# RobotVisionHKA/LiFCal

Measured on AMD Instinct MI355X. Metric: micro-image obs/sec through Jacobian+Schur at 1M obs, higher is better.
Workload: dtype f64; 1 GPU; metric_web: 334 frames, 24720 points, 999994 micro-image observations, window 10, config 0xf06 (2 radial + tangential, mlCenterAdj, Cauchy(0.5), refine poses+points); lens_selection=reference generator (lifcal_mla_project), obs_per_gpu=999994, n_reduced=2021, deterministic=False

## Files before the change

lifcal_amd/csrc/sweep3.hpp:

```cpp
#pragma once

namespace lifcal {

template <int NR, bool TAN, bool ADJ, int WR, class ET = double>
__global__ __launch_bounds__(128 * WR, 2) void k_sweep3(Dev d, double radius, int mode) {
  constexpr bool F32 = sizeof(ET) == 4;
  constexpr int NC = 5 + NR + (TAN ? 2 : 0);
  constexpr int NCC = NC * (NC + 1) / 2;
  constexpr int HV = 6 + 2 * NC + 2;
  constexpr uint32_t LP = 64u * WR;
  constexpr uint32_t NT = 2u * LP;
  static_assert(HV * LP <= V2Lds::zd_for(LP), "hand-off buffer must fit the Z matrix");
  if (radius < 0.0 && d.lm[LM_TERMINATION] != 0.0) return;
  extern __shared__ __attribute__((aligned(16))) double sm[];
  const V2Lds lay(d.v2_nfmax, true, LP);
  const uint32_t NFm = lay.nfm, vlen = 6 * NFm + NCMAX + 3;
  double* Spp = sm; double* Scp = sm + lay.off_cp; double* Scc = sm + lay.off_cc;
  double* vgB = sm + lay.off_vec; double* vhd = vgB + vlen; double* vrhs = vhd + vlen;
  double* Fr = sm + lay.off_fr;
  double* slab = sm + lay.off_slab;
  double* Zd = sm + lay.off_zd;
  double* misc = sm + lay.off_misc;
  uint32_t* pidl = (uint32_t*)(misc + MISC_DOUBLES);
  unsigned short* colinfo = (unsigned short*)(misc + MISC_DOUBLES + 32);
  uint32_t flip = 0;
#ifndef LIFCAL_NO_ROLE_FLIP
  if (WR == 2) flip = (__builtin_amdgcn_s_getreg(6 | (0 << 6) | (7 << 11)) != 0) ? LP : 0u;
#endif
  const uint32_t tid = threadIdx.x ^ flip, lane = tid & 63u, w = tid >> 6;
  const bool role_b = w >= (uint32_t)WR;
  const uint32_t wl = w & (uint32_t)(WR - 1);
  const uint32_t t256 = tid & (LP - 1u);
  const uint32_t b = blockIdx.x;
  const uint32_t flo = d.blk_flo[b], nf = d.blk_nf[b];
  const uint32_t ncol = 6 * nf + NC + 1, ncolp = (ncol + 15u) & ~15u;
  const uint32_t zs = ncolp + 2;
  const CamConsts c = *d.camc;
#ifdef LIFCAL_STAMPS
  unsigned long long st_acc[16] = {0, 0, 0, 0, 0, 0, 0, 0, 0, 0, 0, 0, 0, 0, 0, 0}, st_last = 0;
  if (tid == 0 || tid == LP) { asm volatile("s_memtime %0\n\ts_waitcnt lgkmcnt(0)" : "=s"(st_last) :: "memory"); }
#define STAMPB(i) do { if (tid == LP) { unsigned long long t_; asm volatile("s_memtime %0\n\ts_waitcnt lgkmcnt(0)" : "=s"(t_) :: "memory"); st_acc[i] += t_ - st_last; st_last = t_; } } while (0)
#else
#define STAMPB(i) do { } while (0)
#endif
  const uint32_t ps_begin = d.blk_pass0[b], ps_end = d.blk_pass0[b + 1];
  uint32_t nx_np = 0, nx_si = 0, nx_pt = 0, nx_fp = 0, nx_gid = 0, nx_r[2] = {0, 0};
  uint32_t vz;
  asm volatile("v_mov_b32 %0, 0" : "=v"(vz));
  auto fetch_pass = [&](uint32_t q) {
    nx_np = d.pass_np[q + vz];
    nx_si = d.v2_slot[(size_t)q * LP + t256]; nx_pt = d.v2f_pt[(size_t)q * LP + t256]; nx_gid = d.v2_gidx[(size_t)q * LP + t256];
    nx_r[0] = d.v2_tile_row0[q * WR + wl + vz]; nx_r[1] = d.v2_tile_row0[q * WR + wl + 1 + vz];
    nx_fp = d.v2_passpt[(size_t)q * 64 + (tid & 63u)];
  };
  if (ps_begin < ps_end) fetch_pass(ps_begin);
  { double2* z2 = reinterpret_cast<double2*>(sm); for (uint32_t i = tid; i < lay.off_slab / 2; i += NT) z2[i] = double2{0.0, 0.0}; }
  if (tid == 0 && (lay.off_slab & 1u)) sm[lay.off_slab - 1] = 0.0;
  if (tid < MISC_DOUBLES) misc[tid] = 0.0;
  for (uint32_t cI = tid; cI < ncolp; cI += NT)
    colinfo[cI] = (cI < 6 * nf) ? (unsigned short)(((cI / 6) << 8) | (cI % 6)) : (cI < ncol - 1 ? (unsigned short)(0x8000u | (cI - 6 * nf)) : (unsigned short)0xC000u);

  auto zero_slab = [&]() { for (uint32_t i = tid; i < lay.np_max * SLAB_STRIDE; i += NT) slab[i] = 0.0; };
  auto zero_zd = [&](uint32_t krows) { double2* z2 = reinterpret_cast<double2*>(Zd); for (uint32_t i = tid; i < (krows * zs) / 2; i += NT) z2[i] = double2{0.0, 0.0}; };
  auto z_phase = [&](uint32_t np) {
    const uint32_t nwc = ncol - 1;
    const uint32_t nth = NT / nwc > 0 ? NT / nwc : 1;
    const uint32_t gi = tid / nwc, cidx = tid - gi * nwc;
    if (gi < nth || nwc > NT) {
      for (uint32_t cc0 = cidx; cc0 < nwc; cc0 += (nwc > NT ? NT : nwc * nth)) {
#pragma unroll 4
        for (uint32_t lp = (nwc > NT ? 0 : gi); lp < np; lp += (nwc > NT ? 1 : nth)) {
          const double* acc = slab + lp * SLAB_STRIDE;
          double* z = Zd + (size_t)(3 * lp) * zs + cc0;
          const double w0 = z[0], w1 = z[zs], w2 = z[2 * zs];
          if (cc0 >= 6 * nf) {
            double* ga = d.ptacc + (size_t)pidl[lp] * 36 + 9 + (cc0 - 6 * nf);
            store_stream(ga, w0); store_stream(ga + NCMAX, w1); store_stream(ga + 2 * NCMAX, w2);
          }
          z[0] = acc[0] * w0; z[zs] = acc[1] * w0 + acc[3] * w1; z[2 * zs] = acc[2] * w0 + acc[4] * w1 + acc[5] * w2;
        }
      }
    }
  };
  struct LaneGeom { double R[9], Y[3], Gr[3][3]; };
  auto lane_geom = [&](uint32_t fr, uint32_t pt, LaneGeom& q) {
    const double* ft = d.ft + (size_t)fr * FRAME_STRIDE;
    const double* P = d.pts + 3 * (size_t)pt;
#pragma unroll
    for (int k = 0; k < 9; ++k) q.R[k] = ft[k];
    const double P0 = P[0], P1 = P[1], P2 = P[2];
#pragma unroll
    for (int k = 0; k < 3; ++k) q.Y[k] = q.R[3 * k] * P0 + q.R[3 * k + 1] * P1 + q.R[3 * k + 2] * P2;
    const double c0 = ft[12], s0 = ft[13], n0 = q.R[2], n1 = q.R[5], n2 = q.R[8];
    q.Gr[0][0] = 0.0;     q.Gr[0][1] = c0 * q.Y[2] - s0 * q.Y[1]; q.Gr[0][2] = n1 * q.Y[2] - n2 * q.Y[1];
    q.Gr[1][0] = -q.Y[2]; q.Gr[1][1] = s0 * q.Y[0];               q.Gr[1][2] = n2 * q.Y[0] - n0 * q.Y[2];
    q.Gr[2][0] = q.Y[1];  q.Gr[2][1] = -c0 * q.Y[0];              q.Gr[2][2] = n0 * q.Y[1] - n1 * q.Y[0];
  };
  const uint32_t frs = NFm * lay.nrep;
  struct RunMask { double m1, m2, m4, m8; bool head; };
  auto run_masks = [&](uint32_t cnt, uint32_t lf) {
    const int key = cnt > 0 ? (int)lf : (int)(0x7F000000u + lane);
    RunMask r;
    r.m1 = __builtin_amdgcn_update_dpp(-1, key, 0x101, 0xf, 0xf, false) == key ? 1.0 : 0.0;
    r.m2 = __builtin_amdgcn_update_dpp(-1, key, 0x102, 0xf, 0xf, false) == key ? 1.0 : 0.0;
    r.m4 = __builtin_amdgcn_update_dpp(-1, key, 0x104, 0xf, 0xf, false) == key ? 1.0 : 0.0;
    r.m8 = __builtin_amdgcn_update_dpp(-1, key, 0x108, 0xf, 0xf, false) == key ? 1.0 : 0.0;
    r.head = cnt > 0 && __builtin_amdgcn_update_dpp(-1, key, 0x111, 0xf, 0xf, false) != key;
    return r;
  };
  auto run_sum = [](double v, const RunMask& r) {
    auto shl = [](double x, auto ctrl) {
      const int lo = __double2loint(x), hi = __double2hiint(x);
      return __hiloint2double(__builtin_amdgcn_update_dpp(0, hi, decltype(ctrl)::value, 0xf, 0xf, true),
                              __builtin_amdgcn_update_dpp(0, lo, decltype(ctrl)::value, 0xf, 0xf, true));
    };
    v = fma(shl(v, std::integral_constant<int, 0x101>{}), r.m1, v);
    v = fma(shl(v, std::integral_constant<int, 0x102>{}), r.m2, v);
    v = fma(shl(v, std::integral_constant<int, 0x104>{}), r.m4, v);
    v = fma(shl(v, std::integral_constant<int, 0x108>{}), r.m8, v);
    return v;
  };
  uint32_t* hw_written = (uint32_t*)(misc + 4) + wl;
  uint32_t* hw_read = (uint32_t*)(misc + 4) + 4 + wl;
  uint32_t* eval_done = (uint32_t*)(misc + 3);
  const bool det = d.deterministic != 0;
  uint32_t* turn = (uint32_t*)(misc + 8) + (role_b ? 1 : 0);
  uint32_t my_turn = wl;
  auto wait_for = [](uint32_t* flag, uint32_t need) {
    while (__hip_atomic_load(flag, __ATOMIC_ACQUIRE, __HIP_MEMORY_SCOPE_WORKGROUP) < need) __builtin_amdgcn_s_sleep(2);
  };
  auto publish = [](uint32_t* flag, uint32_t value) {
    asm volatile("s_waitcnt lgkmcnt(0)" ::: "memory");
    __hip_atomic_store(flag, value, __ATOMIC_RELEASE, __HIP_MEMORY_SCOPE_WORKGROUP);
  };

  const uint32_t nmt = (ncol + 3u) >> 2, ntri = nmt * (nmt + 1) / 2;
  auto tri_decode = [](uint32_t t, uint32_t& mi, uint32_t& mj) {
    mi = (uint32_t)((sqrtf(8.0f * (float)t + 1.0f) - 1.0f) * 0.5f);
    while (mi * (mi + 1) / 2 > t) --mi;
    while ((mi + 1) * (mi + 2) / 2 <= t) ++mi;
    mj = t - mi * (mi + 1) / 2;
  };
  auto gemm_tile = [&](uint32_t mi, uint32_t mj, uint32_t kfirst, uint32_t kstep, uint32_t krows, double (&acc16)[4][4]) {
    const double* za = Zd + 4 * mi;
    const double* zb = Zd + 4 * mj;
    double2 cur[4][4];
#pragma unroll
    for (int r = 0; r < 4; ++r) {
      cur[r][0] = *reinterpret_cast<const double2*>(za + (size_t)(kfirst + r) * zs);
      cur[r][1] = *reinterpret_cast<const double2*>(za + (size_t)(kfirst + r) * zs + 2);
      cur[r][2] = *reinterpret_cast<const double2*>(zb + (size_t)(kfirst + r) * zs);
      cur[r][3] = *reinterpret_cast<const double2*>(zb + (size_t)(kfirst + r) * zs + 2);
    }
#pragma unroll 2
    for (uint32_t k0 = kfirst; k0 < krows; k0 += kstep) {
      double2 nxt[4][4];
      const uint32_t kn = (k0 + kstep < krows) ? k0 + kstep : k0;
#pragma unroll
      for (int r = 0; r < 4; ++r) {
        nxt[r][0] = *reinterpret_cast<const double2*>(za + (size_t)(kn + r) * zs);
        nxt[r][1] = *reinterpret_cast<const double2*>(za + (size_t)(kn + r) * zs + 2);
        nxt[r][2] = *reinterpret_cast<const double2*>(zb + (size_t)(kn + r) * zs);
        nxt[r][3] = *reinterpret_cast<const double2*>(zb + (size_t)(kn + r) * zs + 2);
      }
#pragma unroll
      for (int r = 0; r < 4; ++r) {
        const double av[4] = {cur[r][0].x, cur[r][0].y, cur[r][1].x, cur[r][1].y};
        const double bq[4] = {cur[r][2].x, cur[r][2].y, cur[r][3].x, cur[r][3].y};
#pragma unroll
        for (int i = 0; i < 4; ++i)
#pragma unroll
          for (int j = 0; j < 4; ++j) acc16[i][j] += av[i] * bq[j];
      }
#pragma unroll
      for (int r = 0; r < 4; ++r)
#pragma unroll
        for (int q = 0; q < 4; ++q) cur[r][q] = nxt[r][q];
    }
  };
  auto emit_tile = [&](uint32_t mi, uint32_t mj, const double (&acc16)[4][4]) {
#pragma unroll
    for (int i = 0; i < 4; ++i) {
      const uint32_t ci = 4 * mi + i;
      const uint32_t ii = colinfo[ci < ncolp ? ci : 0];
#pragma unroll
      for (int j = 0; j < 4; ++j) {
        const uint32_t cj = 4 * mj + j;
        const double dv = acc16[i][j];
        if (ci >= ncol || cj >= ncol || ci < cj) continue;
        const uint32_t jj = colinfo[cj];
        if (!(ii & 0x8000u)) {
          const uint32_t lfi = ii >> 8, lfj = jj >> 8;
          Spp[(size_t)(lfi * (lfi + 1) / 2 + lfj) * 36 + (ii & 0xFFu) * 6 + (jj & 0xFFu)] -= dv;
        } else if (!(ii & 0x4000u)) {
          const uint32_t jc = ii & 0xFFu;
          if (!(jj & 0x8000u)) Scp[(size_t)jc * 6 * NFm + cj] -= dv;
          else Scc[jc * (jc + 1) / 2 + (jj & 0xFFu)] -= dv;
        } else if (cj < ncol - 1) {
          if (!(jj & 0x8000u)) vrhs[cj] += dv; else vrhs[6 * NFm + (jj & 0xFFu)] += dv;
        }
      }
    }
  };
  const bool keep_tiles = (WR == 4) && (mode == 0) && ntri <= LP;
  const bool ksplit = keep_tiles && lay.has_bt();
  const bool share_tiles = (WR != 4) && (mode == 0);
  double* bt = sm + lay.off_bt;
  if (!role_b) {
    double cost = 0.0, lmant = 1.0; int lexp = 0;
    uint32_t hbase = 0;
    uint32_t passes_done = 0;
    uint32_t mi0 = 0, mj0 = 0;
    if (keep_tiles && tid < ntri) tri_decode(tid, mi0, mj0);
    double tacc[4][4];
#pragma unroll
    for (int i = 0; i < 4; ++i)
#pragma unroll
      for (int j = 0; j < 4; ++j) tacc[i][j] = 0.0;

    STAMP(14);
    for (uint32_t ps = ps_begin; ps < ps_end; ++ps) {
      const uint32_t np = __builtin_amdgcn_readfirstlane(nx_np);
      const uint32_t si = nx_si, pt = nx_pt, fp = nx_fp, gidx = nx_gid;
      const uint32_t row0 = __builtin_amdgcn_readfirstlane(nx_r[0]), kmax = __builtin_amdgcn_readfirstlane(nx_r[1]) - row0;
      if (ps + 1 < ps_end) fetch_pass(ps + 1);
      const uint32_t krows = (3 * np + 7u) & ~7u;
      const uint32_t cnt = si & 0xFFu, lf = (si >> 8) & 0xFFu, lp = (si >> 16) & 0xFFu;
      const uint32_t fr = flo + lf;
      const ET* obs_u = F32 ? reinterpret_cast<const ET*>(d.v2_du) : reinterpret_cast<const ET*>(d.v2_u);
      const ET* obs_v = F32 ? reinterpret_cast<const ET*>(d.v2_dv) : reinterpret_cast<const ET*>(d.v2_v);
      const ET* lens_tab = F32 ? reinterpret_cast<const ET*>(d.ltf) : reinterpret_cast<const ET*>(d.lt);
      double ftv[12], P0, P1, P2;
      {
        const double* ft = d.ft + (size_t)fr * FRAME_STRIDE;
        const double* P = d.pts + 3 * (size_t)pt;
#pragma unroll
        for (int i = 0; i < 12; ++i) ftv[i] = ft[i];
        P0 = P[0]; P1 = P[1]; P2 = P[2];
      }
      ET ua = 0, va = 0, ub = 0, vb = 0; uint32_t lb = 0, la = 0, l0 = 0;
      {
        const size_t at = (size_t)row0 * 64 + lane;
        const size_t at2 = ((size_t)row0 + (kmax > 1 ? 1u : 0u)) * 64 + lane;
        ua = obs_u[at]; va = obs_v[at]; l0 = d.v2_lens[at];
        ub = obs_u[at2]; vb = obs_v[at2]; lb = d.v2_lens[at2];
      }
      STAMP(12);
      zero_slab();
      STAMP(13);
      lds_barrier();
      STAMP(0);
      typename std::conditional<F32, GroupConsts2F, GroupConsts2>::type gcn;
      {
        const double Xc = ftv[0] * P0 + ftv[1] * P1 + ftv[2] * P2 + ftv[9], Yc = ftv[3] * P0 + ftv[4] * P1 + ftv[5] * P2 + ftv[10], Zc = ftv[6] * P0 + ftv[7] * P1 + ftv[8] * P2 + ftv[11];
        if constexpr (F32) group_prepare2f<ADJ>(c, Xc, Yc, Zc, gcn); else group_prepare2<ADJ>(c, Xc, Yc, Zc, gcn);
      }
      double A[6] = {0, 0, 0, 0, 0, 0}, bv[3] = {0, 0, 0};
      ET* hand = reinterpret_cast<ET*>(Zd) + t256;
      constexpr uint32_t HS = LP;
      ET Ln[LENS_STRIDE];
      double wn0 = 0.0, wn1 = 0.0;
      {
        const ET* L = lens_tab + (size_t)l0 * LENS_STRIDE;
#pragma unroll
        for (int i = 0; i < LENS_STRIDE; ++i) Ln[i] = L[i];
        if constexpr (F32) { wn0 = d.ltw[2 * (size_t)l0]; wn1 = d.ltw[2 * (size_t)l0 + 1]; }
      }
      typename std::conditional<F32, CamF, int>::type cf{};
      if constexpr (F32) cf = cam_to_float(c);
      auto step = [&](uint32_t k, ET& uc, ET& vc, uint32_t& lc, const uint32_t ln) {
        wait_for(hw_read, hbase + k);
        if (k < cnt) {
          const ET u = uc, v = vc;
          ET L[LENS_STRIDE];
#pragma unroll
          for (int i = 0; i < LENS_STRIDE; ++i) L[i] = Ln[i];
          ET r[2], Jq[2][3], Jc[2][NC];
          ET arg;
          if constexpr (F32) obs_eval2f_pk<NR, TAN, ADJ>(cf, gcn, L, wn0, wn1, u, v, d.robust != 0, r, Jq, Jc, arg);
          else obs_eval2<NR, TAN, ADJ>(c, gcn, L, u, v, d.robust != 0, r, Jq, Jc, arg);
#pragma unroll
          for (int a = 0; a < 2; ++a) {
#pragma unroll
            for (int j = 0; j < NC; ++j) hand[(6 + a * NC + j) * HS] = Jc[a][j];
#pragma unroll
            for (int i = 0; i < 3; ++i) hand[(a * 3 + i) * HS] = Jq[a][i];
            hand[(6 + 2 * NC + a) * HS] = r[a];
          }
          if (d.robust) { int ex; lmant = frexp(lmant * (double)arg, &ex); lexp += ex; }
          else cost += 0.5 * (double)arg;
#pragma unroll
          for (int a = 0; a < 2; ++a) {
            const double q0 = Jq[a][0], q1 = Jq[a][1], q2 = Jq[a][2], ra = r[a];
            A[0] += q0 * q0; A[1] += q0 * q1; A[2] += q0 * q2;
            A[3] += q1 * q1; A[4] += q1 * q2; A[5] += q2 * q2;
            bv[0] += q0 * ra; bv[1] += q1 * ra; bv[2] += q2 * ra;
          }
        }
        {
          const ET* Lp = lens_tab + (size_t)ln * LENS_STRIDE;
#pragma unroll
          for (int i = 0; i < LENS_STRIDE; ++i) Ln[i] = Lp[i];
          if constexpr (F32) { wn0 = d.ltw[2 * (size_t)ln]; wn1 = d.ltw[2 * (size_t)ln + 1]; }
          const uint32_t kk = (k + 2 < kmax) ? k + 2 : kmax - 1;
          const size_t at = ((size_t)row0 + kk) * 64 + lane;
          uc = obs_u[at]; vc = obs_v[at]; lc = d.v2_lens[at];
        }
        publish(hw_written, hbase + k + 1);
      };
      for (uint32_t k = 0; k < kmax; k += 2) {
        step(k, ua, va, la, lb);
        if (k + 1 < kmax) step(k + 1, ub, vb, lb, la);
      }
      hbase += kmax;
      LaneGeom q;
      { uint32_t fr2 = fr, pt2 = pt; asm volatile("" : "+v"(fr2), "+v"(pt2)); lane_geom(fr2, pt2, q); }
      asm volatile("" :: "v"(nx_si), "v"(nx_pt), "v"(nx_fp), "v"(nx_np), "v"(nx_gid), "v"(nx_r[0]), "v"(nx_r[1]));
      const double fsg0 = d.sigP[3 * (size_t)fp], fsg1 = d.sigP[3 * (size_t)fp + 1], fsg2 = d.sigP[3 * (size_t)fp + 2];
      STAMP(7);
      lds_barrier();
      if (mode == 0) zero_zd(krows);
      lds_barrier();
      asm volatile("" :: "v"(fsg0), "v"(fsg1), "v"(fsg2));
      if (det) wait_for(turn, my_turn);
      if (cnt > 0) {
        const double Am[3][3] = {{A[0], A[1], A[2]}, {A[1], A[3], A[4]}, {A[2], A[4], A[5]}};
        const double (&R)[9] = q.R; const double (&Gr)[3][3] = q.Gr;
        double AG[3][3], GAG[3][3];
#pragma unroll
        for (int i = 0; i < 3; ++i)
#pragma unroll
          for (int j = 0; j < 3; ++j) AG[i][j] = Am[i][0] * Gr[0][j] + Am[i][1] * Gr[1][j] + Am[i][2] * Gr[2][j];
#pragma unroll
        for (int i = 0; i < 3; ++i)
#pragma unroll
          for (int j = 0; j < 3; ++j) GAG[i][j] = Gr[0][i] * AG[0][j] + Gr[1][i] * AG[1][j] + Gr[2][i] * AG[2][j];
        RunMask rm = run_masks(cnt, lf);
        const bool fpose = d.frame_live[fr] != 0;
        rm.head = rm.head && fpose;
        double* fr_acc = Fr + lf;
        {
          int vi = 0;
#pragma unroll
          for (int a = 0; a < 6; ++a)
#pragma unroll
            for (int bb = 0; bb <= a; ++bb) {
              double v;
              if (a < 3) v = GAG[a][bb]; else if (bb < 3) v = AG[a - 3][bb]; else v = Am[a - 3][bb - 3];
              v = run_sum(v, rm);
              if (rm.head) atomicAdd(fr_acc + (size_t)vi * frs, v);
              ++vi;
            }
#pragma unroll
          for (int a = 0; a < 3; ++a) { const double v = run_sum(Gr[0][a] * bv[0] + Gr[1][a] * bv[1] + Gr[2][a] * bv[2], rm); if (rm.head) atomicAdd(fr_acc + (size_t)(21 + a) * frs, v); }
#pragma unroll
          for (int a = 0; a < 3; ++a) { const double v = run_sum(bv[a], rm); if (rm.head) atomicAdd(fr_acc + (size_t)(24 + a) * frs, v); }
        }
        double AR[3][3];
#pragma unroll
        for (int i = 0; i < 3; ++i)
#pragma unroll
          for (int j = 0; j < 3; ++j) AR[i][j] = Am[i][0] * R[j] + Am[i][1] * R[3 + j] + Am[i][2] * R[6 + j];
        double* acc = slab + lp * SLAB_STRIDE;
#pragma unroll
        for (int i = 0; i < 3; ++i) {
#pragma unroll
          for (int j = 0; j <= i; ++j) {
            const double u_ij = R[i] * AR[0][j] + R[3 + i] * AR[1][j] + R[6 + i] * AR[2][j];
            const int pos = (i == 0) ? 0 : (i == 1 ? (j == 0 ? 1 : 3) : (j == 0 ? 2 : (j == 1 ? 4 : 5)));
            atomicAdd(acc + pos, u_ij);
          }
        }
        if (mode == 0) {
          { double* ga = d.Av + (size_t)gidx * 6;
            store_stream(ga, A[0], A[1]); store_stream(ga + 2, A[2], A[3]); store_stream(ga + 4, A[4], A[5]); }
#pragma unroll
          for (int i = 0; i < 3; ++i) {
            atomicAdd(acc + 6 + i, R[i] * bv[0] + R[3 + i] * bv[1] + R[6 + i] * bv[2]);
            double* zrow = Zd + (size_t)(3 * lp + i) * zs + 6 * lf;
            double w6[6];
#pragma unroll
            for (int j = 0; j < 3; ++j) { w6[j] = R[i] * AG[0][j] + R[3 + i] * AG[1][j] + R[6 + i] * AG[2][j]; w6[3 + j] = R[i] * Am[0][j] + R[3 + i] * Am[1][j] + R[6 + i] * Am[2][j]; }
            const bool rot = (lp & 1u) != 0;
#pragma unroll
            for (int jj = 0; jj < 6; ++jj) {
              const double wv = rot ? w6[(jj + 1) % 6] : w6[jj];
              const uint32_t col = rot ? (uint32_t)((jj + 1) % 6) : (uint32_t)jj;
              if (fpose) atomicAdd(zrow + col, wv);
            }
          }
        }
      }
      if (det) { publish(turn, my_turn + 1); my_turn += (uint32_t)WR; }
      STAMP(6);
      asm volatile("s_waitcnt lgkmcnt(0)" ::: "memory");
      if (lane == 0) __hip_atomic_fetch_add(eval_done, 1u, __ATOMIC_RELAXED, __HIP_MEMORY_SCOPE_WORKGROUP);
      ++passes_done;
      if (w == 0) wait_for(eval_done, (uint32_t)WR * passes_done);
      STAMP(1);
      if (tid < np) {
        const uint32_t p = fp;
        pidl[tid] = p;
        double* acc = slab + tid * SLAB_STRIDE;
        double U0 = acc[0], U1 = acc[1], U2 = acc[2], U3 = acc[3], U4 = acc[4], U5 = acc[5];
        if (mode == 1) {
          double* ga = d.ptacc + (size_t)p * 36;
          store_stream(ga, U0); store_stream(ga + 3, U3); store_stream(ga + 5, U5);
        } else {
          const double g0 = acc[6], g1 = acc[7], g2 = acc[8];
          double lam[3];
          {
            const double h[3] = {U0, U3, U5}, sgv[3] = {fsg0, fsg1, fsg2};
#pragma unroll
            for (int k = 0; k < 3; ++k) { const double sg = sgv[k]; lam[k] = fmin(fmax(h[k] * sg * sg, d.lm_min), d.lm_max) / (lm_radius(d, radius) * sg * sg); }
          }
          U0 += lam[0]; U3 += lam[1]; U5 += lam[2];
          bool ok = U0 > 0.0;
          double i00 = rsqrt(U0);
          const double l10 = U1 * i00, l20 = U2 * i00;
          const double d11 = U3 - l10 * l10; ok = ok && (d11 > 0.0);
          double i11 = rsqrt(d11);
          const double l21 = (U4 - l20 * l10) * i11;
          const double d22 = U5 - l20 * l20 - l21 * l21; ok = ok && (d22 > 0.0);
          double i22 = rsqrt(d22);
          double m10 = -l10 * i00 * i11, m21 = -l21 * i11 * i22, m20 = -(l20 * i00 + l21 * m10) * i22;
          if (!ok) { i00 = i11 = i22 = m10 = m21 = m20 = 0.0; atomicAdd(misc + 1, 1.0); }
          double* gu = d.Uinv + 9 * (size_t)p;
          const double v00 = i00 * i00 + m10 * m10 + m20 * m20, v01 = m10 * i11 + m20 * m21, v02 = m20 * i22;
          const double v11 = i11 * i11 + m21 * m21, v12 = m21 * i22, v22 = i22 * i22;
          {
            const double vu[9] = {v00, v01, v02, v01, v11, v12, v02, v12, v22};
#pragma unroll
            for (int k = 0; k < 9; ++k) store_stream(gu + k, vu[k]);
          }
          double* gl = d.lamP + 3 * (size_t)p;
          double* ga = d.ptacc + (size_t)p * 36 + 6;
#pragma unroll
          for (int k = 0; k < 3; ++k) store_stream(gl + k, lam[k]);
          store_stream(ga, g0); store_stream(ga + 1, g1); store_stream(ga + 2, g2);
          const double gm = fmax(fabs(g0), fmax(fabs(g1), fabs(g2)));
          atomicMax((unsigned long long*)(misc + 2), (unsigned long long)__double_as_longlong(gm));
          acc[0] = i00; acc[1] = m10; acc[2] = m20; acc[3] = i11; acc[4] = m21; acc[5] = i22;
          double* z0 = Zd + (size_t)(3 * tid) * zs + (ncol - 1);
          z0[0] = i00 * g0; z0[zs] = m10 * g0 + i11 * g1; z0[2 * zs] = m20 * g0 + m21 * g1 + i22 * g2;
        }
      }
      lds_barrier();
      STAMP(2);
      if (mode == 0) {
        z_phase(np);
        lds_barrier();
        STAMP(3);
        if (keep_tiles) {
          if (tid < ntri) gemm_tile(mi0, mj0, 0, ksplit ? 8u : 4u, krows, tacc);
        } else {
          for (uint32_t t = tid; t < ntri; t += (share_tiles ? NT : LP)) {
            uint32_t mi, mj; tri_decode(t, mi, mj);
            double acc16[4][4];
#pragma unroll
            for (int i = 0; i < 4; ++i)
#pragma unroll
              for (int j = 0; j < 4; ++j) acc16[i][j] = 0.0;
            gemm_tile(mi, mj, 0, 4, krows, acc16);
            emit_tile(mi, mj, acc16);
          }
        }
      }
      lds_barrier();
      STAMP(4);
    }
    STAMP(8);
    if (keep_tiles && tid < ntri) {
      if (ksplit) {
#pragma unroll
        for (int i = 0; i < 4; ++i)
#pragma unroll
          for (int j = 0; j < 4; ++j) tacc[i][j] += bt[(i * 4 + j) * LP + tid];
      }
      uint32_t ci4[4], cj4[4];
#pragma unroll
      for (int i = 0; i < 4; ++i) { const uint32_t ci = 4 * mi0 + i, cj = 4 * mj0 + i; ci4[i] = colinfo[ci < ncolp ? ci : 0]; cj4[i] = colinfo[cj < ncolp ? cj : 0]; }
      uint32_t off[4][4]; double sg[4][4];
      const uint32_t dummy = lay.off_zd + 1024u + tid;
#pragma unroll
      for (int i = 0; i < 4; ++i)
#pragma unroll
        for (int j = 0; j < 4; ++j) {
          const uint32_t ci = 4 * mi0 + i, cj = 4 * mj0 + j, ii = ci4[i], jj = cj4[j];
          uint32_t o = dummy; double sgn = -1.0;
          if (!(ci >= ncol || cj >= ncol || ci < cj)) {
            if (!(ii & 0x8000u)) {
              const uint32_t lfi = ii >> 8, lfj = jj >> 8;
              o = (lfi * (lfi + 1) / 2 + lfj) * 36 + (ii & 0xFFu) * 6 + (jj & 0xFFu);
            } else if (!(ii & 0x4000u)) {
              const uint32_t jc = ii & 0xFFu;
              o = !(jj & 0x8000u) ? lay.off_cp + jc * 6 * NFm + cj : lay.off_cc + jc * (jc + 1) / 2 + (jj & 0xFFu);
            } else if (cj < ncol - 1) {
              o = lay.off_vec + 2 * vlen + (!(jj & 0x8000u) ? cj : 6 * NFm + (jj & 0xFFu));
              sgn = 1.0;
            }
          }
          off[i][j] = o; sg[i][j] = sgn;
        }
      double oldv[4][4];
#pragma unroll
      for (int i = 0; i < 4; ++i)
#pragma unroll
        for (int j = 0; j < 4; ++j) oldv[i][j] = sm[off[i][j]];
#pragma unroll
      for (int i = 0; i < 4; ++i)
#pragma unroll
        for (int j = 0; j < 4; ++j) sm[off[i][j]] = oldv[i][j] + sg[i][j] * tacc[i][j];
    }
    STAMP(9);
    if (d.robust) cost += 0.5 * c.loss_b * (log(lmant) + (double)lexp * 0.6931471805599453);
    cost = wave_sum_dpp(cost);
    if (det) wait_for(turn, my_turn);
    if (lane == 63) atomicAdd(misc + 0, cost);
    if (det) publish(turn, my_turn + 1);
    lds_barrier(); lds_barrier();
  } else {
    double cc[NCC], gc[NC];
    uint32_t hbase = 0;
#pragma unroll
    for (int i = 0; i < NCC; ++i) cc[i] = 0.0;
#pragma unroll
    for (int i = 0; i < NC; ++i) gc[i] = 0.0;
    for (uint32_t ps = ps_begin; ps < ps_end; ++ps) {
      const uint32_t np = __builtin_amdgcn_readfirstlane(nx_np);
      const uint32_t si = nx_si, pt = nx_pt;
      const uint32_t kmax = __builtin_amdgcn_readfirstlane(nx_r[1]) - __builtin_amdgcn_readfirstlane(nx_r[0]);
      if (ps + 1 < ps_end) fetch_pass(ps + 1);
      const uint32_t krows = (3 * np + 7u) & ~7u;
      zero_slab();
      lds_barrier();
      STAMPB(0);
      const uint32_t cnt = si & 0xFFu, lf = (si >> 8) & 0xFFu, lp = (si >> 16) & 0xFFu;
      double C[3][NC];
#pragma unroll
      for (int i = 0; i < 3; ++i)
#pragma unroll
        for (int j = 0; j < NC; ++j) C[i][j] = 0.0;
      const ET* hand = reinterpret_cast<const ET*>(Zd) + t256;
      constexpr uint32_t HS = LP;
      for (uint32_t k = 0; k < kmax; ++k) {
        wait_for(hw_written, hbase + k + 1);
        const bool live = k < cnt;
#pragma unroll
        for (int a = 0; a < 2; ++a) {
          double r = 0.0, Jq[3] = {0.0, 0.0, 0.0}, Jc[NC];
#pragma unroll
          for (int j = 0; j < NC; ++j) Jc[j] = 0.0;
          if (live) {
#pragma unroll
            for (int i = 0; i < 3; ++i) Jq[i] = hand[(a * 3 + i) * HS];
#pragma unroll
            for (int j = 0; j < NC; ++j) Jc[j] = hand[(6 + a * NC + j) * HS];
            r = hand[(6 + 2 * NC + a) * HS];
          }
          if (a == 1) publish(hw_read, hbase + k + 1);
          if (live) {
#pragma unroll
            for (int i = 0; i < 3; ++i)
#pragma unroll
              for (int j = 0; j < NC; ++j) C[i][j] += Jq[i] * Jc[j];
            int t = 0;
#pragma unroll
            for (int i = 0; i < NC; ++i) {
              gc[i] += Jc[i] * r;
#pragma unroll
              for (int j = 0; j <= i; ++j) cc[t++] += Jc[i] * Jc[j];
            }
          }
        }
      }
      hbase += kmax;
      asm volatile("" :: "v"(nx_si), "v"(nx_pt), "v"(nx_np), "v"(nx_r[0]), "v"(nx_r[1]));
      LaneGeom q;
      STAMPB(1);
      lane_geom(flo + lf, pt, q);
      lds_barrier();
      if (mode == 0) zero_zd(krows);
      lds_barrier();
      STAMPB(2);
      if (det) wait_for(turn, my_turn);
      if (mode == 0 && cnt > 0) {
        const double (&R)[9] = q.R; const double (&Gr)[3][3] = q.Gr;
#pragma unroll
        for (int i = 0; i < 3; ++i)
#pragma unroll
          for (int j = 0; j < NC; ++j) C[i][j] *= c.chm[j];
        RunMask rm = run_masks(cnt, lf);
        rm.head = rm.head && d.frame_live[flo + lf] != 0;
        double* fr_acc = Fr + lf;
#pragma unroll
        for (int j = 0; j < NC; ++j) {
#pragma unroll
          for (int ci = 0; ci < 3; ++ci) { const double v = run_sum(C[0][j] * Gr[0][ci] + C[1][j] * Gr[1][ci] + C[2][j] * Gr[2][ci], rm); if (rm.head) atomicAdd(fr_acc + (size_t)(27 + j * 6 + ci) * frs, v); }
#pragma unroll
          for (int ci = 0; ci < 3; ++ci) { const double v = run_sum(C[ci][j], rm); if (rm.head) atomicAdd(fr_acc + (size_t)(27 + j * 6 + 3 + ci) * frs, v); }
        }
#pragma unroll
        for (int i = 0; i < 3; ++i) {
          double* zrow = Zd + (size_t)(3 * lp + i) * zs + 6 * nf;
          double wc[NC];
#pragma unroll
          for (int j = 0; j < NC; ++j) wc[j] = R[i] * C[0][j] + R[3 + i] * C[1][j] + R[6 + i] * C[2][j];
          const bool rot = (lp & 1u) != 0;
#pragma unroll
          for (int jj = 0; jj < NC; ++jj) atomicAdd(zrow + (rot ? (uint32_t)((jj + 1) % NC) : (uint32_t)jj), rot ? wc[(jj + 1) % NC] : wc[jj]);
        }
      }
      if (det) { publish(turn, my_turn + 1); my_turn += (uint32_t)WR; }
      STAMPB(3);
      lds_barrier();
      STAMPB(4);
      if (mode == 0) {
        z_phase(np);
        lds_barrier();
      }
      if (ksplit && t256 < ntri) {
        uint32_t mi, mj; tri_decode(t256, mi, mj);
        double acc16[4][4];
#pragma unroll
        for (int i = 0; i < 4; ++i)
#pragma unroll
          for (int j = 0; j < 4; ++j) acc16[i][j] = bt[(i * 4 + j) * LP + t256];
        gemm_tile(mi, mj, 4, 8, krows, acc16);
#pragma unroll
        for (int i = 0; i < 4; ++i)
#pragma unroll
          for (int j = 0; j < 4; ++j) bt[(i * 4 + j) * LP + t256] = acc16[i][j];
      }
      if (share_tiles) {
        for (uint32_t t = tid; t < ntri; t += NT) {
          uint32_t mi, mj; tri_decode(t, mi, mj);
          double acc16[4][4];
#pragma unroll
          for (int i = 0; i < 4; ++i)
#pragma unroll
            for (int j = 0; j < 4; ++j) acc16[i][j] = 0.0;
          gemm_tile(mi, mj, 0, 4, krows, acc16);
          emit_tile(mi, mj, acc16);
        }
      }
      lds_barrier();
      STAMPB(5);
    }
    {
      int t = 0;
#pragma unroll
      for (int i = 0; i < NC; ++i) {
        gc[i] *= c.chm[i];
#pragma unroll
        for (int j = 0; j <= i; ++j) cc[t++] *= c.chm[i] * c.chm[j];
      }
    }
    constexpr int NVB = NCC + NC;
    constexpr uint32_t NROWS = 4u * WR;
    {
      double* red = Zd;
      const uint32_t rowi = t256 >> 4;
      const bool tail = (lane & 15u) == 15u;
#pragma unroll
      for (int idx = 0; idx < NVB; ++idx) {
        double v = (idx < NCC) ? cc[idx < NCC ? idx : 0] : gc[(idx - NCC) >= 0 && (idx - NCC) < NC ? idx - NCC : 0];
        v = dpp_add_step<0x111, 0xf>(v); v = dpp_add_step<0x112, 0xf>(v); v = dpp_add_step<0x114, 0xf>(v); v = dpp_add_step<0x118, 0xf>(v);
        if (tail) red[rowi * NVB + idx] = v;
      }
      lds_barrier();
      if (t256 < (uint32_t)NVB) {
        const int idx = (int)t256;
        double sacc = 0.0;
#pragma unroll
        for (uint32_t k = 0; k < NROWS; ++k) sacc += red[k * NVB + idx];
        if (idx < NCC) {
          int i = 0; while ((i + 1) * (i + 2) / 2 <= idx) ++i;
          if (mode == 0) Scc[idx] += sacc;
          if (idx == i * (i + 1) / 2 + i) vhd[6 * NFm + i] += sacc;
        } else {
          vgB[6 * NFm + (idx - NCC)] += sacc;
        }
      }
      lds_barrier();
    }
  }
  lds_barrier();
  STAMP(10);
  if (!det) {
    if (mode == 0) {
      double* hr = d.hot + (size_t)(b % HOT_ROWS) * HOT_STRIDE;
      if (tid < (uint32_t)NCC) atomicAdd(hr + tid, Scc[tid]);
      if (tid < (uint32_t)NC) {
        atomicAdd(hr + NCC + tid, vhd[6 * NFm + tid]);
        atomicAdd(hr + NCC + NC + tid, vgB[6 * NFm + tid]);
        atomicAdd(hr + NCC + 2 * NC + tid, vrhs[6 * NFm + tid]);
      }
      if (tid == 0) {
        atomicAdd(hr + NCC + 3 * NC, misc[0]);
        if (misc[1] != 0.0) atomicAdd(d.scal + SCAL_BAD_U, misc[1]);
        atomicMax((unsigned long long*)(hr + NCC + 3 * NC + 1), *(unsigned long long*)(misc + 2));
      }
    } else if (tid < (uint32_t)NC) {
      atomicAdd(d.hdiag + 6 * d.F + 3 * d.Q + tid, vhd[6 * NFm + tid]);
    }
  }
  for (uint32_t i = tid; i < FRV * nf; i += NT) {
    const uint32_t v = i / nf, lf = i % nf;
    double sacc = 0.0;
    for (uint32_t r = 0; r < lay.nrep; ++r) sacc += Fr[(size_t)v * NFm * lay.nrep + r * NFm + lf];
    if (v < 21) {
      uint32_t a = 0; while ((a + 1) * (a + 2) / 2 <= v) ++a;
      const uint32_t bb = v - a * (a + 1) / 2;
      Spp[(size_t)(lf * (lf + 1) / 2 + lf) * 36 + a * 6 + bb] += sacc;
      if (a == bb) vhd[6 * lf + a] += sacc;
    } else if (v < 27) {
      vgB[6 * lf + (v - 21)] += sacc;
    } else if (mode == 0 && v < 27 + 6 * (uint32_t)NC) {
      const uint32_t j = (v - 27) / 6, ci = (v - 27) % 6;
      Scp[(size_t)j * 6 * NFm + 6 * lf + ci] += sacc;
    }
  }
  lds_barrier();
  STAMP(11);
  if (det) {
    double* out = d.det_slab + (size_t)b * d.det_stride;
    for (uint32_t i = tid; i < lay.off_fr; i += NT) out[i] = sm[i];
    if (tid < 3) out[lay.off_fr + tid] = misc[tid];
    return;
  }
  const uint32_t camrow = 3 * d.Q;
  for (uint32_t i = tid; i < 6 * nf; i += NT) atomicAdd(d.hdiag + 6 * flo + i, vhd[i]);
  if (mode == 0) {
    for (uint32_t i = tid; i < 6 * nf; i += NT) { atomicAdd(d.gB + 6 * flo + i, vgB[i]); atomicAdd(d.rhsacc + 6 * flo + i, vrhs[i]); }
    for (uint32_t i = tid; i < (uint32_t)NC * 6 * nf; i += NT) {
      const uint32_t j = i / (6 * nf), cidx = i % (6 * nf);
      atomicAdd(d.Sarrow + (size_t)(camrow + j) * d.ld + 6 * flo + cidx, Scp[(size_t)j * 6 * NFm + cidx]);
    }
    const uint32_t npp = nf * (nf + 1) / 2;
    for (uint32_t i = tid; i < npp * 36; i += NT) {
      const uint32_t blk = i / 36, e = i % 36;
      uint32_t a = (uint32_t)((sqrtf(8.0f * (float)blk + 1.0f) - 1.0f) * 0.5f);
      while (a * (a + 1) / 2 > blk) --a;
      while ((a + 1) * (a + 2) / 2 <= blk) ++a;
      const uint32_t bb = blk - a * (a + 1) / 2, dd = a - bb;
      const double v = Spp[i];
      if (dd <= d.bw && v != 0.0 && !(dd == 0 && (e % 6) > (e / 6))) atomicAdd(d.Sband + ((size_t)(flo + a) * (d.bw + 1) + dd) * 36 + e, v);
    }
  }
#ifdef LIFCAL_STAMPS
  lds_barrier();
  STAMP(5);
  if ((tid == 0 || tid == LP) && d.dbg) for (int i = 0; i < 16; ++i) d.dbg[(size_t)b * 32 + (tid == 0 ? 0 : 16) + i] = st_acc[i];
#endif
}

}
```

Baseline: 10.08 billion obs/s.

## Split pass into point-factor then pose-column scatter, applying Cholesky factor at scatter time

Restructures each pass so that the point Hessian blocks are accumulated first. Wave 0 then factors the point blocks and publishes a flag, while the other waves continue with the frame-run reductions. In non-deterministic mode the pose columns of Z are scattered already multiplied by the inverse Cholesky factor, so z_phase only has to transform the camera-intrinsic columns rather than every pose column. This is meant to remove most of the post-barrier z_phase work and overlap the factorization with the frame accumulation. In exchange it adds a second flag wait per pass and more atomics per observation, and the deterministic path gets extra turn handoffs.

```diff
diff --git a/lifcal_amd/csrc/sweep3.hpp b/lifcal_amd/csrc/sweep3.hpp
--- a/lifcal_amd/csrc/sweep3.hpp
+++ b/lifcal_amd/csrc/sweep3.hpp
@@ -63,23 +63,24 @@
   auto zero_slab = [&]() { for (uint32_t i = tid; i < lay.np_max * SLAB_STRIDE; i += NT) slab[i] = 0.0; };
   auto zero_zd = [&](uint32_t krows) { double2* z2 = reinterpret_cast<double2*>(Zd); for (uint32_t i = tid; i < (krows * zs) / 2; i += NT) z2[i] = double2{0.0, 0.0}; };
   auto z_phase = [&](uint32_t np) {
-    const uint32_t nwc = ncol - 1;
-    const uint32_t nth = NT / nwc > 0 ? NT / nwc : 1;
-    const uint32_t gi = tid / nwc, cidx = tid - gi * nwc;
-    if (gi < nth || nwc > NT) {
-      for (uint32_t cc0 = cidx; cc0 < nwc; cc0 += (nwc > NT ? NT : nwc * nth)) {
-#pragma unroll 4
-        for (uint32_t lp = (nwc > NT ? 0 : gi); lp < np; lp += (nwc > NT ? 1 : nth)) {
-          const double* acc = slab + lp * SLAB_STRIDE;
-          double* z = Zd + (size_t)(3 * lp) * zs + cc0;
-          const double w0 = z[0], w1 = z[zs], w2 = z[2 * zs];
-          if (cc0 >= 6 * nf) {
-            double* ga = d.ptacc + (size_t)pidl[lp] * 36 + 9 + (cc0 - 6 * nf);
-            store_stream(ga, w0); store_stream(ga + NCMAX, w1); store_stream(ga + 2 * NCMAX, w2);
-          }
-          z[0] = acc[0] * w0; z[zs] = acc[1] * w0 + acc[3] * w1; z[2 * zs] = acc[2] * w0 + acc[4] * w1 + acc[5] * w2;
-        }
-      }
+    if (d.deterministic != 0) {
+      const uint32_t npc = 6 * nf;
+      for (uint32_t i = tid; i < npc * np; i += NT) {
+        const uint32_t lp = i / npc, cc0 = i - lp * npc;
+        const double* acc = slab + lp * SLAB_STRIDE;
+        double* z = Zd + (size_t)(3 * lp) * zs + cc0;
+        const double w0 = z[0], w1 = z[zs], w2 = z[2 * zs];
+        z[0] = acc[0] * w0; z[zs] = acc[1] * w0 + acc[3] * w1; z[2 * zs] = acc[2] * w0 + acc[4] * w1 + acc[5] * w2;
+      }
+    }
+    for (uint32_t i = tid; i < (uint32_t)NC * np; i += NT) {
+      const uint32_t lp = i / (uint32_t)NC, jc = i - lp * (uint32_t)NC;
+      const double* acc = slab + lp * SLAB_STRIDE;
+      double* z = Zd + (size_t)(3 * lp) * zs + 6 * nf + jc;
+      const double w0 = z[0], w1 = z[zs], w2 = z[2 * zs];
+      double* ga = d.ptacc + (size_t)pidl[lp] * 36 + 9 + jc;
+      store_stream(ga, w0); store_stream(ga + NCMAX, w1); store_stream(ga + 2 * NCMAX, w2);
+      z[0] = acc[0] * w0; z[zs] = acc[1] * w0 + acc[3] * w1; z[2 * zs] = acc[2] * w0 + acc[4] * w1 + acc[5] * w2;
     }
   };
   struct LaneGeom { double R[9], Y[3], Gr[3][3]; };
@@ -132,6 +133,55 @@
   auto publish = [](uint32_t* flag, uint32_t value) {
     asm volatile("s_waitcnt lgkmcnt(0)" ::: "memory");
     __hip_atomic_store(flag, value, __ATOMIC_RELEASE, __HIP_MEMORY_SCOPE_WORKGROUP);
+  };
+  uint32_t* factor_done = (uint32_t*)(misc + 3) + 1;
+  auto factor_points = [&](uint32_t np, uint32_t p, double fsg0, double fsg1, double fsg2) {
+    if (tid < np) {
+      pidl[tid] = p;
+      double* acc = slab + tid * SLAB_STRIDE;
+      double U0 = acc[0], U1 = acc[1], U2 = acc[2], U3 = acc[3], U4 = acc[4], U5 = acc[5];
+      if (mode == 1) {
+        double* ga = d.ptacc + (size_t)p * 36;
+        store_stream(ga, U0); store_stream(ga + 3, U3); store_stream(ga + 5, U5);
+      } else {
+        const double g0 = acc[6], g1 = acc[7], g2 = acc[8];
+        double lam[3];
+        {
+          const double h[3] = {U0, U3, U5}, sgv[3] = {fsg0, fsg1, fsg2};
+#pragma unroll
+          for (int k = 0; k < 3; ++k) { const double sg = sgv[k]; lam[k] = fmin(fmax(h[k] * sg * sg, d.lm_min), d.lm_max) / (lm_radius(d, radius) * sg * sg); }
+        }
+        U0 += lam[0]; U3 += lam[1]; U5 += lam[2];
+        bool ok = U0 > 0.0;
+        double i00 = rsqrt(U0);
+        const double l10 = U1 * i00, l20 = U2 * i00;
+        const double d11 = U3 - l10 * l10; ok = ok && (d11 > 0.0);
+        double i11 = rsqrt(d11);
+        const double l21 = (U4 - l20 * l10) * i11;
+        const double d22 = U5 - l20 * l20 - l21 * l21; ok = ok && (d22 > 0.0);
+        double i22 = rsqrt(d22);
+        double m10 = -l10 * i00 * i11, m21 = -l21 * i11 * i22, m20 = -(l20 * i00 + l21 * m10) * i22;
+        if (!ok) { i00 = i11 = i22 = m10 = m21 = m20 = 0.0; atomicAdd(misc + 1, 1.0); }
+        double* gu = d.Uinv + 9 * (size_t)p;
+        const double v00 = i00 * i00 + m10 * m10 + m20 * m20, v01 = m10 * i11 + m20 * m21, v02 = m20 * i22;
+        const double v11 = i11 * i11 + m21 * m21, v12 = m21 * i22, v22 = i22 * i22;
+        {
+          const double vu[9] = {v00, v01, v02, v01, v11, v12, v02, v12, v22};
+#pragma unroll
+          for (int k = 0; k < 9; ++k) store_stream(gu + k, vu[k]);
+        }
+        double* gl = d.lamP + 3 * (size_t)p;
+        double* ga = d.ptacc + (size_t)p * 36 + 6;
+#pragma unroll
+        for (int k = 0; k < 3; ++k) store_stream(gl + k, lam[k]);
+        store_stream(ga, g0); store_stream(ga + 1, g1); store_stream(ga + 2, g2);
+        const double gm = fmax(fabs(g0), fmax(fabs(g1), fabs(g2)));
+        atomicMax((unsigned long long*)(misc + 2), (unsigned long long)__double_as_longlong(gm));
+        acc[0] = i00; acc[1] = m10; acc[2] = m20; acc[3] = i11; acc[4] = m21; acc[5] = i22;
+        double* z0 = Zd + (size_t)(3 * tid) * zs + (ncol - 1);
+        z0[0] = i00 * g0; z0[zs] = m10 * g0 + i11 * g1; z0[2 * zs] = m20 * g0 + m21 * g1 + i22 * g2;
+      }
+    }
   };
 
   const uint32_t nmt = (ncol + 3u) >> 2, ntri = nmt * (nmt + 1) / 2;
@@ -322,21 +372,58 @@
       if (mode == 0) zero_zd(krows);
       lds_barrier();
       asm volatile("" :: "v"(fsg0), "v"(fsg1), "v"(fsg2));
+      const double Am[3][3] = {{A[0], A[1], A[2]}, {A[1], A[3], A[4]}, {A[2], A[4], A[5]}};
+      const double (&R)[9] = q.R; const double (&Gr)[3][3] = q.Gr;
+      double* acc = slab + lp * SLAB_STRIDE;
       if (det) wait_for(turn, my_turn);
       if (cnt > 0) {
-        const double Am[3][3] = {{A[0], A[1], A[2]}, {A[1], A[3], A[4]}, {A[2], A[4], A[5]}};
-        const double (&R)[9] = q.R; const double (&Gr)[3][3] = q.Gr;
-        double AG[3][3], GAG[3][3];
+        double AR[3][3];
 #pragma unroll
         for (int i = 0; i < 3; ++i)
 #pragma unroll
-          for (int j = 0; j < 3; ++j) AG[i][j] = Am[i][0] * Gr[0][j] + Am[i][1] * Gr[1][j] + Am[i][2] * Gr[2][j];
+          for (int j = 0; j < 3; ++j) AR[i][j] = Am[i][0] * R[j] + Am[i][1] * R[3 + j] + Am[i][2] * R[6 + j];
+#pragma unroll
+        for (int i = 0; i < 3; ++i) {
+#pragma unroll
+          for (int j = 0; j <= i; ++j) {
+            const double u_ij = R[i] * AR[0][j] + R[3 + i] * AR[1][j] + R[6 + i] * AR[2][j];
+            const int pos = (i == 0) ? 0 : (i == 1 ? (j == 0 ? 1 : 3) : (j == 0 ? 2 : (j == 1 ? 4 : 5)));
+            atomicAdd(acc + pos, u_ij);
+          }
+        }
+        if (mode == 0) {
+          { double* ga = d.Av + (size_t)gidx * 6;
+            store_stream(ga, A[0], A[1]); store_stream(ga + 2, A[2], A[3]); store_stream(ga + 4, A[4], A[5]); }
+#pragma unroll
+          for (int i = 0; i < 3; ++i) atomicAdd(acc + 6 + i, R[i] * bv[0] + R[3 + i] * bv[1] + R[6 + i] * bv[2]);
+        }
+      }
+      if (det) publish(turn, my_turn + 1);
+      STAMP(6);
+      asm volatile("s_waitcnt lgkmcnt(0)" ::: "memory");
+      if (lane == 0) __hip_atomic_fetch_add(eval_done, 1u, __ATOMIC_RELAXED, __HIP_MEMORY_SCOPE_WORKGROUP);
+      ++passes_done;
+      if (w == 0) {
+        wait_for(eval_done, (uint32_t)WR * passes_done);
+        STAMP(1);
+        factor_points(np, fp, fsg0, fsg1, fsg2);
+        publish(factor_done, passes_done);
+        STAMP(2);
+      }
+      if (det) wait_for(turn, my_turn + (uint32_t)WR);
+      const bool fpose = cnt > 0 && d.frame_live[fr] != 0;
+      double AG[3][3];
+#pragma unroll
+      for (int i = 0; i < 3; ++i)
+#pragma unroll
+        for (int j = 0; j < 3; ++j) AG[i][j] = Am[i][0] * Gr[0][j] + Am[i][1] * Gr[1][j] + Am[i][2] * Gr[2][j];
+      if (cnt > 0) {
+        double GAG[3][3];
 #pragma unroll
         for (int i = 0; i < 3; ++i)
 #pragma unroll
           for (int j = 0; j < 3; ++j) GAG[i][j] = Gr[0][i] * AG[0][j] + Gr[1][i] * AG[1][j] + Gr[2][i] * AG[2][j];
         RunMask rm = run_masks(cnt, lf);
-        const bool fpose = d.frame_live[fr] != 0;
         rm.head = rm.head && fpose;
         double* fr_acc = Fr + lf;
         {
@@ -356,97 +443,37 @@
 #pragma unroll
           for (int a = 0; a < 3; ++a) { const double v = run_sum(bv[a], rm); if (rm.head) atomicAdd(fr_acc + (size_t)(24 + a) * frs, v); }
         }
-        double AR[3][3];
-#pragma unroll
-        for (int i = 0; i < 3; ++i)
-#pragma unroll
-          for (int j = 0; j < 3; ++j) AR[i][j] = Am[i][0] * R[j] + Am[i][1] * R[3 + j] + Am[i][2] * R[6 + j];
-        double* acc = slab + lp * SLAB_STRIDE;
-#pragma unroll
-        for (int i = 0; i < 3; ++i) {
-#pragma unroll
-          for (int j = 0; j <= i; ++j) {
-            const double u_ij = R[i] * AR[0][j] + R[3 + i] * AR[1][j] + R[6 + i] * AR[2][j];
-            const int pos = (i == 0) ? 0 : (i == 1 ? (j == 0 ? 1 : 3) : (j == 0 ? 2 : (j == 1 ? 4 : 5)));
-            atomicAdd(acc + pos, u_ij);
+      }
+      if (mode == 0) {
+        if (!det) wait_for(factor_done, passes_done);
+        if (fpose) {
+          double i00 = 1.0, m10 = 0.0, m20 = 0.0, i11 = 1.0, m21 = 0.0, i22 = 1.0;
+          if (!det) { i00 = acc[0]; m10 = acc[1]; m20 = acc[2]; i11 = acc[3]; m21 = acc[4]; i22 = acc[5]; }
+          double* zcol = Zd + (size_t)(3 * lp) * zs + 6 * lf;
+          const bool rot = (lp & 1u) != 0;
+#pragma unroll
+          for (int jj = 0; jj < 6; ++jj) {
+            const int ja = jj, jb = (jj + 1) % 6;
+            double x[3];
+#pragma unroll
+            for (int k = 0; k < 3; ++k) {
+              const double xa = ja < 3 ? AG[k][ja % 3] : Am[k][ja % 3], xb = jb < 3 ? AG[k][jb % 3] : Am[k][jb % 3];
+              x[k] = rot ? xb : xa;
+            }
+            const uint32_t col = rot ? (uint32_t)jb : (uint32_t)ja;
+            const double w0 = R[0] * x[0] + R[3] * x[1] + R[6] * x[2];
+            const double w1 = R[1] * x[0] + R[4] * x[1] + R[7] * x[2];
+            const double w2 = R[2] * x[0] + R[5] * x[1] + R[8] * x[2];
+            atomicAdd(zcol + col, i00 * w0);
+            atomicAdd(zcol + zs + col, m10 * w0 + i11 * w1);
+            atomicAdd(zcol + 2 * zs + col, m20 * w0 + m21 * w1 + i22 * w2);
           }
         }
-        if (mode == 0) {
-          { double* ga = d.Av + (size_t)gidx * 6;
-            store_stream(ga, A[0], A[1]); store_stream(ga + 2, A[2], A[3]); store_stream(ga + 4, A[4], A[5]); }
-#pragma unroll
-          for (int i = 0; i < 3; ++i) {
-            atomicAdd(acc + 6 + i, R[i] * bv[0] + R[3 + i] * bv[1] + R[6 + i] * bv[2]);
-            double* zrow = Zd + (size_t)(3 * lp + i) * zs + 6 * lf;
-            double w6[6];
-#pragma unroll
-            for (int j = 0; j < 3; ++j) { w6[j] = R[i] * AG[0][j] + R[3 + i] * AG[1][j] + R[6 + i] * AG[2][j]; w6[3 + j] = R[i] * Am[0][j] + R[3 + i] * Am[1][j] + R[6 + i] * Am[2][j]; }
-            const bool rot = (lp & 1u) != 0;
-#pragma unroll
-            for (int jj = 0; jj < 6; ++jj) {
-              const double wv = rot ? w6[(jj + 1) % 6] : w6[jj];
-              const uint32_t col = rot ? (uint32_t)((jj + 1) % 6) : (uint32_t)jj;
-              if (fpose) atomicAdd(zrow + col, wv);
-            }
-          }
-        }
-      }
-      if (det) { publish(turn, my_turn + 1); my_turn += (uint32_t)WR; }
+      }
+      if (det) { publish(turn, my_turn + (uint32_t)WR + 1); my_turn += 2u * (uint32_t)WR; }
       STAMP(6);
-      asm volatile("s_waitcnt lgkmcnt(0)" ::: "memory");
-      if (lane == 0) __hip_atomic_fetch_add(eval_done, 1u, __ATOMIC_RELAXED, __HIP_MEMORY_SCOPE_WORKGROUP);
-      ++passes_done;
-      if (w == 0) wait_for(eval_done, (uint32_t)WR * passes_done);
-      STAMP(1);
-      if (tid < np) {
-        const uint32_t p = fp;
-        pidl[tid] = p;
-        double* acc = slab + tid * SLAB_STRIDE;
-        double U0 = acc[0], U1 = acc[1], U2 = acc[2], U3 = acc[3], U4 = acc[4], U5 = acc[5];
-        if (mode == 1) {
-          double* ga = d.ptacc + (size_t)p * 36;
-          store_stream(ga, U0); store_stream(ga + 3, U3); store_stream(ga + 5, U5);
-        } else {
-          const double g0 = acc[6], g1 = acc[7], g2 = acc[8];
-          double lam[3];
-          {
-            const double h[3] = {U0, U3, U5}, sgv[3] = {fsg0, fsg1, fsg2};
-#pragma unroll
-            for (int k = 0; k < 3; ++k) { const double sg = sgv[k]; lam[k] = fmin(fmax(h[k] * sg * sg, d.lm_min), d.lm_max) / (lm_radius(d, radius) * sg * sg); }
-          }
-          U0 += lam[0]; U3 += lam[1]; U5 += lam[2];
-          bool ok = U0 > 0.0;
-          double i00 = rsqrt(U0);
-          const double l10 = U1 * i00, l20 = U2 * i00;
-          const double d11 = U3 - l10 * l10; ok = ok && (d11 > 0.0);
-          double i11 = rsqrt(d11);
-          const double l21 = (U4 - l20 * l10) * i11;
-          const double d22 = U5 - l20 * l20 - l21 * l21; ok = ok && (d22 > 0.0);
-          double i22 = rsqrt(d22);
-          double m10 = -l10 * i00 * i11, m21 = -l21 * i11 * i22, m20 = -(l20 * i00 + l21 * m10) * i22;
-          if (!ok) { i00 = i11 = i22 = m10 = m21 = m20 = 0.0; atomicAdd(misc + 1, 1.0); }
-          double* gu = d.Uinv + 9 * (size_t)p;
-          const double v00 = i00 * i00 + m10 * m10 + m20 * m20, v01 = m10 * i11 + m20 * m21, v02 = m20 * i22;
-          const double v11 = i11 * i11 + m21 * m21, v12 = m21 * i22, v22 = i22 * i22;
-          {
-            const double vu[9] = {v00, v01, v02, v01, v11, v12, v02, v12, v22};
-#pragma unroll
-            for (int k = 0; k < 9; ++k) store_stream(gu + k, vu[k]);
-          }
-          double* gl = d.lamP + 3 * (size_t)p;
-          double* ga = d.ptacc + (size_t)p * 36 + 6;
-#pragma unroll
-          for (int k = 0; k < 3; ++k) store_stream(gl + k, lam[k]);
-          store_stream(ga, g0); store_stream(ga + 1, g1); store_stream(ga + 2, g2);
-          const double gm = fmax(fabs(g0), fmax(fabs(g1), fabs(g2)));
-          atomicMax((unsigned long long*)(misc + 2), (unsigned long long)__double_as_longlong(gm));
-          acc[0] = i00; acc[1] = m10; acc[2] = m20; acc[3] = i11; acc[4] = m21; acc[5] = i22;
-          double* z0 = Zd + (size_t)(3 * tid) * zs + (ncol - 1);
-          z0[0] = i00 * g0; z0[zs] = m10 * g0 + i11 * g1; z0[2 * zs] = m20 * g0 + m21 * g1 + i22 * g2;
-        }
-      }
-      lds_barrier();
-      STAMP(2);
+      lds_barrier();
+      STAMP(15);
       if (mode == 0) {
         z_phase(np);
         lds_barrier();
```

After: 10.64 billion obs/s (median of 6 runs). 5.5% higher.
